# EnzoCording/FleetRL

Measured on AMD Instinct MI355X. Metric: env-steps/sec (num_envs x EVs batch, 1 launch per step), higher is better.
Workload: dtype f64

## Files before the change

### fleetrl_amd/_capi.py

```python
from __future__ import annotations

import ctypes as C
import os

import numpy as np

ABI_VERSION = 11

OK, ERR_INVALID, ERR_HIP, ERR_STATE, ERR_NODEVICE, ERR_UNSUPPORTED = 0, 1, 2, 3, 4, 5
DEG_NONE, DEG_LINEAR, DEG_RAINFLOW = 0, 1, 2
PICK_STATIC, PICK_RANDOM, PICK_EVAL = 0, 1, 2
ACT_F32, ACT_F64 = 0, 1
LAUNCH_EAGER, LAUNCH_GRAPH, LAUNCH_DIRECT, LAUNCH_DIRECT_ONE_QUEUE = 0, 1, 2, 3
POLICY_UNCONTROLLED, POLICY_DISTRIBUTED, POLICY_NIGHT = 2, 3, 4
LP_UNREACHABLE, LP_NEG_RETURN, LP_ABOVE_TARGET, LP_GRID_NEGATIVE = 1, 2, 4, 8

DEVERR_OBS_FORMAT, DEVERR_NEG_LIFE, DEVERR_SOH_MISMATCH, DEVERR_DOD_RANGE, DEVERR_TABLE_END, DEVERR_INTERNAL, DEVERR_PLACEMENT = 1, 2, 4, 8, 16, 32, 64

FIELDS = {
    "soc": (0, np.float64, True),
    "hours_left": (1, np.float32, True),
    "soh": (2, np.float64, True),
    "soc_deg": (3, np.float64, True),
    "target_soc": (4, np.float64, True),
# ... 516 lines not shown
    lib.fleet_rccl_comm_create.argtypes = [C.c_int, C.c_int, C.c_int, vp, C.POINTER(vp)]
    lib.fleet_rccl_comm_destroy.argtypes = [vp]
    lib.fleet_gather_episode_stats_rccl.argtypes = [vp, vp, C.c_int, vp]
    if hasattr(lib, "fleet_direct_queues"):
        lib.fleet_direct_queues.argtypes = [vp]
        lib.fleet_direct_queues.restype = C.c_int
    if hasattr(lib, "fleet_direct_placement"):
        lib.fleet_direct_placement.argtypes = [vp, C.POINTER(C.c_int32), C.POINTER(C.c_int32), C.POINTER(C.c_int32)]
        lib.fleet_direct_split_plan.argtypes = [C.c_uint32, C.c_int, C.POINTER(C.c_uint32)]
        lib.fleet_debug_direct_fault.argtypes = [vp, C.c_int, C.c_int]
        for name in ("fleet_direct_placement", "fleet_direct_split_plan", "fleet_debug_direct_fault"):
            getattr(lib, name).restype = C.c_int
    if hasattr(lib, "fleet_step_instance"):
        lib.fleet_step_instance.argtypes = [C.c_int] * 8 + [C.c_char_p, C.c_size_t, C.POINTER(C.c_uint32)]
        lib.fleet_step_instance.restype = C.c_int
        lib.fleet_max_evs_per_lane_group.argtypes = []
        lib.fleet_max_evs_per_lane_group.restype = C.c_int
    if hasattr(lib, "fleet_set_direct_state_only"):
        lib.fleet_set_direct_state_only.argtypes = [vp, C.c_int]
        lib.fleet_direct_packet_counts.argtypes = [vp, C.POINTER(C.c_uint64), C.POINTER(C.c_uint64)]
        lib.fleet_step_has_state_only.argtypes = [C.c_int] * 8 + [C.POINTER(C.c_int32)]
        for name in ("fleet_set_direct_state_only", "fleet_direct_packet_counts", "fleet_step_has_state_only"):
            getattr(lib, name).restype = C.c_int
    if hasattr(lib, "fleet_selftest_stress"):
        lib.fleet_selftest_stress.argtypes = [C.c_int, C.c_uint64, C.c_uint64, C.POINTER(C.c_double)]
        lib.fleet_selftest_stress.restype = C.c_int
    if hasattr(lib, "fleet_selftest_division"):
        lib.fleet_selftest_division.argtypes = [C.c_int, C.c_uint64, C.c_uint64, C.POINTER(C.c_uint64)]
        lib.fleet_selftest_division.restype = C.c_int
    lib.fleet_state_layout.argtypes = [C.POINTER(FleetParams), C.POINTER(FleetStateLayout)]
    lib.fleet_state_table_hash.argtypes = [C.POINTER(FleetParams), C.POINTER(FleetTablesC), C.POINTER(C.c_uint64)]
    lib.fleet_state_check.argtypes = [C.POINTER(FleetParams), C.c_uint64, vp, C.c_uint64]
    lib.fleet_state_bytes.argtypes = [vp, C.POINTER(C.c_uint64)]
    for name in ("fleet_state_save_dev", "fleet_state_load_dev", "fleet_state_save_host", "fleet_state_load_host"):
        getattr(lib, name).argtypes = [vp, vp, C.c_uint64]
    lib.fleet_fork_envs.argtypes = [vp, vp, vp, vp, C.c_int]
    for name in STATE_SYMBOLS:
        getattr(lib, name).restype = C.c_int
    dp = C.POINTER(C.c_double)
    lib.fleet_norm_create.argtypes = [C.c_int, C.POINTER(FleetNormParams), C.POINTER(vp)]
    lib.fleet_norm_destroy.argtypes = [vp]
    lib.fleet_norm_last_error.argtypes = [vp]
    lib.fleet_norm_set_stream.argtypes = [vp, vp]
    lib.fleet_norm_configure.argtypes = [vp, C.POINTER(FleetNormParams)]
    lib.fleet_norm_reset_dev.argtypes = [vp, f32p, f32p]
    lib.fleet_norm_step_dev.argtypes = [vp, f32p, f64p, u8p, f32p, f32p, f64p, f32p]
# ... 227 lines not shown
SACTRAIN_SYMBOLS = ("fleet_sactrain_create", "fleet_sactrain_destroy", "fleet_sactrain_last_error", "fleet_sactrain_describe",
                    "fleet_sactrain_alpha_dev", "fleet_sactrain_scale_dev", "fleet_sactrain_polyak_dev", "fleet_sactrain_sac_dev")

COLLECT_SYMBOLS = ("fleet_collect_create", "fleet_collect_destroy", "fleet_collect_last_error", "fleet_collect_describe",
                   "fleet_collect_reset_dev", "fleet_collect_ppo_dev", "fleet_collect_offpolicy_dev", "fleet_collect_episodes_dev",
                   "fleet_collect_finish_dev", "fleet_collect_episodes_read")

EVAL_SYMBOLS = ("fleet_eval_create", "fleet_eval_destroy", "fleet_eval_last_error", "fleet_eval_describe", "fleet_eval_sync_norm_dev",
                "fleet_eval_run_dev", "fleet_eval_episodes_dev", "fleet_eval_clear_dev", "fleet_eval_best_load_dev", "fleet_eval_best_export_dev",
                "fleet_eval_episodes_read")

EXPORTED_SYMBOLS = (
    "fleet_obs_dim", "fleet_create", "fleet_destroy", "fleet_last_error", "fleet_set_stream", "fleet_get_stream", "fleet_use_own_stream",
    "fleet_synchronize", "fleet_stream_query", "fleet_log_capacity", "fleet_log_dropped", "fleet_log_read", "fleet_log_clear",
    "fleet_log_summary_dev", "fleet_set_start_schedule", "fleet_reset_dev", "fleet_step_dev", "fleet_step_many_dev", "fleet_rollout_policy_dev",
    "fleet_set_night_policy", "fleet_reset_host",
    "fleet_step_host", "fleet_get", "fleet_get_dev", "fleet_get_dist_factor", "fleet_check_errors", "fleet_timer_start",
    "fleet_timer_stop", "fleet_timer_mark", "fleet_timer_read", "fleet_run_tape_dev", "fleet_time_steps_dev",
    "fleet_host_alloc", "fleet_host_free", "fleet_last_step_episodes", "fleet_last_step_error_bits",
    "fleet_time_regions_begin", "fleet_time_regions_read", "fleet_rccl_unique_id", "fleet_rccl_comm_create",
    "fleet_rccl_comm_destroy", "fleet_gather_episode_stats_rccl", "fleet_selftest_division", "fleet_direct_queues", "fleet_selftest_stress",
    "fleet_direct_placement", "fleet_direct_split_plan", "fleet_debug_direct_fault", "fleet_set_rainflow_count_all",
    "fleet_lp_plan_dev", "fleet_step_instance", "fleet_max_evs_per_lane_group",
    "fleet_set_direct_state_only", "fleet_direct_packet_counts", "fleet_step_has_state_only",
) + NORM_SYMBOLS + STATE_SYMBOLS + ROLLOUT_SYMBOLS + REPLAY_SYMBOLS + POLICY_SYMBOLS + EXPLORE_SYMBOLS + NOISE_SYMBOLS + QTARGET_SYMBOLS + PPO_SYMBOLS + TD3_SYMBOLS + ADAM_SYMBOLS + TRAIN_SYMBOLS + OFFPOLICY_SYMBOLS + SAC_SYMBOLS + COLLECT_SYMBOLS + EVAL_SYMBOLS


def step_instance(num_envs: int, num_cars: int, deg_mode: int, real_time: bool, log_data: bool, act_mode: int = ACT_F32, K: int = 1,
                  has_done_count: bool = False) -> tuple[str, int]:
    name = C.create_string_buffer(64)
    grid = C.c_uint32()
    rc = load_library().fleet_step_instance(int(num_envs), int(num_cars), int(deg_mode), int(bool(real_time)), int(bool(log_data)),
                                            int(act_mode), int(K), int(bool(has_done_count)), name, len(name), C.byref(grid))
    if rc != OK:
        raise FleetHipError(rc, "fleet_step_instance: argument out of range")
    return name.value.decode(), int(grid.value)


def step_has_state_only(num_envs: int, num_cars: int, deg_mode: int, real_time: bool, log_data: bool, act_mode: int = ACT_F32, K: int = 1,
                        has_done_count: bool = False) -> bool:
    out = C.c_int32()
    rc = load_library().fleet_step_has_state_only(int(num_envs), int(num_cars), int(deg_mode), int(bool(real_time)), int(bool(log_data)),
                                                  int(act_mode), int(K), int(bool(has_done_count)), C.byref(out))
    if rc != OK:
        raise FleetHipError(rc, "fleet_step_has_state_only: argument out of range")
    return bool(out.value)

# ... 116 lines not shown
```

### fleetrl_amd/batch.py

```python
from __future__ import annotations

import ctypes as C

import numpy as np

from . import _capi
from ._capi import FleetHipError

__all__ = ["FleetBatch", "FleetHipError"]


class _PinnedBuffer:

    _dead: list = []

    def __init__(self, lib, nbytes: int):
        out = C.c_void_p()
        rc = lib.fleet_host_alloc(int(nbytes), C.byref(out))
        if rc != _capi.OK or not out.value:
            raise FleetHipError(rc, "fleet_host_alloc failed")
        self._lib, self.address, self.nbytes = lib, int(out.value), int(nbytes)

    def array(self, shape, dtype) -> np.ndarray:
        raw = (C.c_char * self.nbytes).from_address(self.address)
# ... 244 lines not shown
    def set_rainflow_count_all(self, on: bool = True):
        self._check(self.lib.fleet_set_rainflow_count_all(self.h, 1 if on else 0))

    def run_tape_dev(self, steps: int, tape_ptr: int, tape_len: int, obs_ptr: int, reward_ptr: int, done_ptr: int,
                     use_graph: bool = True, act_dtype: int = _capi.ACT_F32):
        self._check(self.lib.fleet_run_tape_dev(self.h, int(steps), tape_ptr, int(tape_len), act_dtype, obs_ptr,
                                                 reward_ptr, done_ptr, int(use_graph)))

    def direct_placement(self):
        m = (C.c_int32 * 8)()
        nx, ag = C.c_int32(), C.c_int32()
        self._check(self.lib.fleet_direct_placement(self.h, m, C.byref(nx), C.byref(ag)))
        return [int(x) for x in m], int(nx.value), bool(ag.value)

    def debug_direct_fault(self, kind: int, tape_row: int):
        self._check(self.lib.fleet_debug_direct_fault(self.h, int(kind), int(tape_row)))

    def direct_queues(self) -> int:
        return int(self.lib.fleet_direct_queues(self.h)) if hasattr(self.lib, "fleet_direct_queues") else 0

    def set_direct_state_only(self, on: bool = True):
        self._check(self.lib.fleet_set_direct_state_only(self.h, 1 if on else 0))

    def direct_packet_counts(self) -> tuple[int, int]:
        live, dead = C.c_uint64(), C.c_uint64()
        self._check(self.lib.fleet_direct_packet_counts(self.h, C.byref(live), C.byref(dead)))
        return int(live.value), int(dead.value)

    def time_steps_dev(self, steps: int, tape_ptr: int, tape_len: int, obs_ptr: int, reward_ptr: int, done_ptr: int,
                       act_dtype: int = _capi.ACT_F32) -> np.ndarray:
        ms = np.zeros(int(steps), dtype=np.float32)
        self._check(self.lib.fleet_time_steps_dev(self.h, int(steps), tape_ptr, int(tape_len), act_dtype, obs_ptr,
                                                   reward_ptr, done_ptr, ms.ctypes.data))
        return ms

    def time_regions_begin(self, regions: int, steps: int, tape_ptr: int, tape_len: int, obs_ptr: int, reward_ptr: int, done_ptr: int,
                           use_graph: bool = True, act_dtype: int = _capi.ACT_F32):
        self._n_regions = int(regions)
        self._check(self.lib.fleet_time_regions_begin(self.h, int(regions), int(steps), tape_ptr, int(tape_len), act_dtype, obs_ptr,
                                                       reward_ptr, done_ptr, int(use_graph)))

    def time_regions_read(self) -> np.ndarray:
        ms = np.zeros(self._n_regions, dtype=np.float32)
        self._check(self.lib.fleet_time_regions_read(self.h, ms.ctypes.data))
        return ms

# ... 89 lines not shown
```

### fleetrl_amd/csrc/fleet_batch.h

```cpp
#pragma once
#include <hip/hip_runtime.h>
#include <stdint.h>

#include <string>
#include <tuple>
#include <vector>

#include "fleet_device.h"
#include "fleet_direct.h"
#include "fleet_state.h"

struct TapeKey {
  const void* tape = nullptr;
  int len = 0, dtype = 0;
  float* obs = nullptr;
  float* term = nullptr;
  double* reward = nullptr;
  uint8_t* done = nullptr;
  int mode = 0;
  uint64_t gen = 0;
  bool operator==(const TapeKey& o) const {
    return std::tie(tape, len, dtype, obs, term, reward, done, mode, gen) ==
           std::tie(o.tape, o.len, o.dtype, o.obs, o.term, o.reward, o.done, o.mode, o.gen);
  }
// ... 31 lines not shown
  char* pin_small = nullptr;
  void* pin_actions = nullptr;
  float* pin_term = nullptr;
  char* pin_obs = nullptr;
  static constexpr int kObsPieces = 3;
  hipEvent_t obs_piece_ev[kObsPieces] = {};
  bool host_step_has_episodes = false;
  uint32_t last_step_err = 0;
  double* st_dist = nullptr;
  int32_t* dev_sched = nullptr;
  FleetCold cold_host{};
  FleetCold* cold_dev = nullptr;
  FleetDev* self_dev = nullptr;
  void* st_field = nullptr;
  hipEvent_t ev_start = nullptr, ev_stop = nullptr;
  std::vector<hipEvent_t> region_events;
  hipGraphExec_t graph_exec = nullptr;
  TapeKey graph_key;
  FleetDirect* direct = nullptr;
  TapeKey dq_key;
  bool dq_timed = false;
  std::vector<double> dq_spans_us;
  bool direct_state_only = true;
  uint64_t gen = 1;
  void* lp_scratch = nullptr;
  size_t lp_scratch_bytes = 0;
  void* logsum_scratch = nullptr;
  uint64_t table_hash = 0;
  FleetStateHeader* pin_state_hdr = nullptr;
  FleetForkScratch fork;
};

inline int direct_drain(FleetEnvBatch* h) {
  if (!h || !h->direct) return FLEET_OK;
  return fleet_direct_wait(h->direct, &h->dq_spans_us, &h->error);
}
#define FLEET_ENTER(h)                          \
  do {                                          \
    const int _rc = direct_drain(h);            \
    if (_rc != FLEET_OK) return _rc;            \
  } while (0)

#define HIP_TRY(b, expr)                                                                         \
  do {                                                                                           \
    hipError_t _e = (expr);                                                                      \
    if (_e != hipSuccess) {                                                                      \
// ... 40 lines not shown
```

### fleetrl_amd/csrc/fleet_capi.hip

```cpp
#include <algorithm>
#include <cstdio>
#include <cstring>

#include "fleet_batch.h"
#include "fleet_logsum.h"
#include "fleet_lp.h"

static thread_local std::string g_create_error;

static const char* deverr_names(uint32_t bits, char* buf, size_t n) {
  snprintf(buf, n, "%s%s%s%s%s%s%s",
           (bits & FLEET_DEVERR_PLACEMENT) ? " placement: a workgroup of a run on the library's own queue ran on another die than probed, the run's results are void;" : "",
           (bits & FLEET_DEVERR_INTERNAL) ? " internal: inconsistent launch arguments;" : "",
           (bits & FLEET_DEVERR_OBS_FORMAT) ? " observation format not recognized;" : "",
           (bits & FLEET_DEVERR_NEG_LIFE) ? " life degradation is negative;" : "",
           (bits & FLEET_DEVERR_SOH_MISMATCH) ? " degradation calculation is not correct;" : "",
           (bits & FLEET_DEVERR_DOD_RANGE) ? " DoD too large;" : "",
           (bits & FLEET_DEVERR_TABLE_END) ? " the episode runs past the last table row;" : "");
  return buf;
}

void fleet_set_create_error(const std::string& why) { g_create_error = why; }

template <typename Edit>
static int push_cold(fleet_handle h, Edit edit) {
  h->gen += 1;
  HIP_TRY(h, hipSetDevice(h->device));
  HIP_TRY(h, hipStreamSynchronize(h->stream));
  const int rc = edit();
  if (rc != FLEET_OK) return rc;
  HIP_TRY(h, hipMemcpy(h->cold_dev, &h->cold_host, sizeof(FleetCold), hipMemcpyHostToDevice));
  return FLEET_OK;
}

extern "C" {

int fleet_obs_dim(const FleetParams* p) {
  if (!p || p->num_cars < 1) return -1;
  return fleet_obs_dim_of(p);
}

int fleet_create(const FleetParams* p, const FleetTables* t, int device, fleet_handle* out) {
  if (out) *out = nullptr;
  if (const char* why = fleet_validate(p, t)) {
    g_create_error = why;
    return FLEET_ERR_INVALID;
  }
  if (!out) {
    g_create_error = "null output handle";
    return FLEET_ERR_INVALID;
  }
  FleetEnvBatch* b = new FleetEnvBatch();
  int rc = fleet_create_impl(p, t, device, b);
// ... 82 lines not shown
  return push_cold(h, [&]() -> int {
    if (h->dev_sched) {
      (void)hipFree(h->dev_sched);
      h->dev_sched = nullptr;
    }
    h->cold_host.sched = nullptr;
    h->cold_host.sched_n = 0;
    if (n_episodes > 0) {
      const size_t n = (size_t)n_episodes * h->d.E;
      for (size_t i = 0; i < n; ++i)
        if (starts[i] < 0 || starts[i] > h->d.T - 1) {
          h->error = "start row outside the table";
          return FLEET_ERR_INVALID;
        }
      HIP_TRY(h, hipMalloc((void**)&h->dev_sched, n * sizeof(int32_t)));
      HIP_TRY(h, hipMemcpy(h->dev_sched, starts, n * sizeof(int32_t), hipMemcpyHostToDevice));
      h->cold_host.sched = h->dev_sched;
      h->cold_host.sched_n = n_episodes;
    }
    return FLEET_OK;
  });
}

int fleet_reset_dev(fleet_handle h, const uint8_t* mask, float* obs) {
  FLEET_ENTER(h);
  if (!h || !obs) return FLEET_ERR_INVALID;
  HIP_TRY(h, hipSetDevice(h->device));
  HIP_TRY(h, fleet_launch_reset(h->d, mask, obs, h->stream));
  return FLEET_OK;
}

int fleet_step_dev(fleet_handle h, const void* actions, int act_dtype, float* obs, double* reward, uint8_t* done,
                   float* terminal_obs) {
  FLEET_ENTER(h);
  if (!h || !actions || !obs || !reward || !done || !act_dtype_ok(act_dtype)) {
    if (h) h->error = "fleet_step_dev: null buffer or bad action dtype";
    return FLEET_ERR_INVALID;
  }
  HIP_TRY(h, hipSetDevice(h->device));
  HIP_TRY(h, fleet_launch_step(h->d, actions, act_dtype, 1, obs, reward, done, terminal_obs, nullptr, h->stream));
  return FLEET_OK;
}

int fleet_step_many_dev(fleet_handle h, int K, const void* actions, int act_dtype, float* obs, double* reward_sum,
                        int32_t* done_count) {
  FLEET_ENTER(h);
// ... 298 lines not shown
    char names[400], buf[640];
    snprintf(buf, sizeof buf, "%s: the handle has device error bits raised (0x%x:%s) and its state is not saved or forked", who, any,
             deverr_names(any, names, sizeof names));
    h->error = buf;
    return FLEET_ERR_STATE;
  }
  return FLEET_OK;
}

static int state_save(fleet_handle h, void* blob, uint64_t bytes, bool host) {
  FLEET_ENTER(h);
  if (!h) return FLEET_ERR_INVALID;
  HIP_TRY(h, hipSetDevice(h->device));
  if (!h->pin_state_hdr) HIP_TRY(h, hipHostMalloc((void**)&h->pin_state_hdr, sizeof(FleetStateHeader), hipHostMallocDefault));
  const int rc = state_clean(h, host ? "fleet_state_save_host" : "fleet_state_save_dev");
  if (rc != FLEET_OK) return rc;
  return fleet_state_save(state_refs(h), blob, bytes, host);
}

static int state_load(fleet_handle h, const void* blob, uint64_t bytes, bool host) {
  FLEET_ENTER(h);
  if (!h) return FLEET_ERR_INVALID;
  HIP_TRY(h, hipSetDevice(h->device));
  const int rc = fleet_state_load(state_refs(h), blob, bytes, host);
  if (rc != FLEET_OK) return rc;
  h->gen += 1;
  h->host_step_has_episodes = false;
  h->last_step_err = 0;
  return FLEET_OK;
}

int fleet_state_bytes(fleet_handle h, uint64_t* bytes) {
  if (!h || !bytes) return FLEET_ERR_INVALID;
  *bytes = fleet_state_blob_bytes(state_refs(h));
  return FLEET_OK;
}
int fleet_state_save_dev(fleet_handle h, void* blob_dev, uint64_t bytes) { return state_save(h, blob_dev, bytes, false); }
int fleet_state_save_host(fleet_handle h, void* blob_host, uint64_t bytes) { return state_save(h, blob_host, bytes, true); }
int fleet_state_load_dev(fleet_handle h, const void* blob_dev, uint64_t bytes) { return state_load(h, blob_dev, bytes, false); }
int fleet_state_load_host(fleet_handle h, const void* blob_host, uint64_t bytes) { return state_load(h, blob_host, bytes, true); }

int fleet_fork_envs(fleet_handle dst, fleet_handle src, const int32_t* dst_idx_host, const int32_t* src_idx_host, int n) {
  FLEET_ENTER(dst);
  if (!dst || !src) return FLEET_ERR_INVALID;
  if (src != dst) {
    const int rc = direct_drain(src);
    if (rc != FLEET_OK) {
      dst->error = "fleet_fork_envs: the source handle: " + src->error;
      return rc;
    }
  }
  if (dst->device != src->device) {
    dst->error = "fleet_fork_envs: the two handles are on different devices";
    return FLEET_ERR_INVALID;
  }
  if (dst->d.log_pos || src->d.log_pos) {
    dst->error = "fleet_fork_envs: a handle with the data log on is not forked (log_data = 1)";
    return FLEET_ERR_UNSUPPORTED;
  }
  HIP_TRY(dst, hipSetDevice(dst->device));
  int rc = state_clean(dst, "fleet_fork_envs");
  if (rc != FLEET_OK) return rc;
  if (src != dst && (rc = state_clean(src, "fleet_fork_envs")) != FLEET_OK) {
    dst->error = src->error;
    return rc;
  }
  return fleet_state_fork(state_refs(dst), state_refs(src), src == dst, dst_idx_host, src_idx_host, n, &dst->fork);
}

}

static int selftest_run(int device, uint64_t n, uint64_t seed, void* out, size_t words,
                        hipError_t (*launch)(unsigned long long, unsigned long long, unsigned long long*, hipStream_t)) {
  if (!out || n == 0) return FLEET_ERR_INVALID;
  int ndev = 0;
  if (hipGetDeviceCount(&ndev) != hipSuccess || ndev <= 0) return FLEET_ERR_NODEVICE;
  if (device < 0 || device >= ndev) return FLEET_ERR_INVALID;
  if (hipSetDevice(device) != hipSuccess) return FLEET_ERR_HIP;
  unsigned long long* dev = nullptr;
  unsigned long long host[2] = {0, 0};
  const size_t bytes = words * sizeof host[0];
  if (hipMalloc(&dev, bytes) != hipSuccess) return FLEET_ERR_HIP;
  int rc = FLEET_OK;
  if (hipMemset(dev, 0, bytes) != hipSuccess || launch(n, seed, dev, nullptr) != hipSuccess ||
      hipMemcpy(host, dev, bytes, hipMemcpyDeviceToHost) != hipSuccess)
    rc = FLEET_ERR_HIP;
  (void)hipFree(dev);
  memcpy(out, host, bytes);
  return rc;
}
// ... 9 lines not shown
```

### fleetrl_amd/csrc/fleet_device.h

```cpp
#pragma once
#include <hip/hip_runtime.h>
#include <stdint.h>

#include "../../include/fleet_hip.h"

struct PhysRow {
  double k_cost;
  double k_rev;
  double k_charge;
  double k_discharge;
  double load;
  double pv;
  double pv_share;
  uint32_t flags_next;
  uint32_t pad;
  double dt;
};

struct SegRec {
  double sor;
  uint32_t tlx;
  uint32_t se;
};
#define SEG_RAW 0x40000000u
// ... 82 lines not shown
  double fd_cyc;
  double fd_cal;
  double sei_l;
  double sei_soh;
};
struct FleetCold {
  double min_laxity, def_soc, init_soh, temperature, dt;
  double batt_cap_nominal, hn_denominator, max_soc, max_hours_needed, max_laxity;
  double inv_max_soc, inv_max_hours_needed, inv_max_laxity;
  unsigned long long seed;
  int picker_mode, start_lo, start_hi, env_id_offset;
  int sched_n;
  int normalize;
  const int32_t* sched;
  const int32_t* pick_rows;
  const uint16_t* tab_hm;
  int32_t* night_start;
  int night_hour, night_minute;
  int night_limit_s;
  int step_s;
  const int32_t* tab_last_deg;
  int32_t* last_len;
  int rf_count_all;
};
#define FLEET_NIGHT_IDLE INT32_MIN

struct FleetDev {
  int E, N, T;
  int obs_dim;
  int episode_steps;
  int stack_cap;
  int tail_a_len;
  int tail_b_len;
  int tail_stride;
  int aux, normalize, is_caretaker, deg_mode, auto_reset;
  int real_time;
  int carry_run;
  double dt, p_avail, init_cap, eta_c, eta_d, penalty_invalid, penalty_oc, clip_oc, target_soc, target_soc_lunch, eps,
      fully_charged_reward, evse_power, grid_connection, penalty_overload, max_time_left, stress_temp;
  double hn_scale;
  double inv_eta_c;
  const SegRec* seg;
  const PhysRow* tab_phys;
  const uint8_t* tab_flags;
  const float* tab_tail;
  const int32_t* tab_finish;
  const FleetCold* cold;
  const struct FleetDev* self;
  Hot* hot;
  SegRec* run;
  double* soh;
  double* soc_deg;
  SeiRec* sei;
  EnvRec* env;
  uint32_t* err_any;
  int log_cap;
  int32_t* log_pos;
  int32_t* log_row;
  double* log_env;
  double* log_ev;
  float* log_obs;
  double* rf_rows;
  int rf_row_stride;
};

hipError_t fleet_launch_reset(const FleetDev& d, const uint8_t* mask, float* obs, hipStream_t s);
hipError_t fleet_launch_step(const FleetDev& d, const void* actions, int act_dtype, int K, float* obs, double* reward,
                             uint8_t* done, float* terminal_obs, int32_t* done_count, hipStream_t s);
struct FleetStepLaunch {
  const void* host_fn;
  const void* host_fn_dead;
  unsigned grid, block, args_bytes;
  unsigned actions_offset[2];
  unsigned packed_n_offset;
  unsigned guard_offset;
  unsigned rec_offset;
  unsigned dead_offset;
  alignas(8) unsigned char args[640];
};
struct FleetStepInstance {
  int G, deg;
  bool multi, wide, log, a64;
  int mode;
};
int fleet_describe_step_instance(const FleetDev& d, int act_mode, int K, bool has_done_count, char* name, size_t name_bytes,
                                 unsigned* grid);
// ... 11 lines not shown
```

### fleetrl_amd/csrc/fleet_kernels.hip

```cpp
#include "fleet_device.h"
#include <cstddef>

#include "fleet_stamps.h"

namespace {

constexpr int kSingleWaves = 4, kMultiWaves = 4, kMultiWideWaves = 2;
#ifndef FLEET_KBLOCK
#define FLEET_KBLOCK 256
#endif
constexpr int kBlock = FLEET_KBLOCK;
constexpr int kMaxGroup = 256;
static_assert(kMaxGroup <= kBlock && kBlock % 64 == 0, "a lane group is a whole number of a workgroup's wavefronts");

}

#include "fleet_wave.h"
#include "fleet_obs.h"
#include "fleet_rainflow.h"
#include "fleet_reset.h"

namespace {

template <int DEG, bool WIDE>
// ... 267 lines not shown
    night_st = d.cold->night_start[e];
    if (G >= 64) night_st = __builtin_amdgcn_readfirstlane(night_st);
  }

  static_assert(!LOG || MULTI, "the data log is compiled into the multi-step kernel only");
  constexpr bool log_on = LOG;
  int lp = log_on ? d.log_pos[e] : 0;
  if (G >= 64) lp = __builtin_amdgcn_readfirstlane(lp);

  const bool rt = kRt && (d.real_time != 0);
  constexpr bool kRfCarry = MULTI && !WIDE && DEG == FLEET_DEG_RAINFLOW;
  RfAccHead acc_c = {0.0, 0, 0};
  RfTop top_c = {0.0, 0.0};
  auto carry_load = [&]() {
    const EvIx i0 = {(size_t)e * N, (unsigned)(g < N ? g : N - 1)};
    const double* row = rf_row_of(d, i0);
    acc_c = *reinterpret_cast<const RfAccHead*>(row);
    top_c = *reinterpret_cast<const RfTop*>(row + 2);
  };
  if (kRfCarry) carry_load();
  double last_rew = 0.0;
  bool last_done = false;
  uint32_t head_after = 0;
  bool head_reset = false;
  for (int k = 0; rt || k < steps; ++k) {
    const int t = r.t;
    int t1 = t + 1;
    if (t1 > d.T - 1) { t1 = d.T - 1; err |= FLEET_DEVERR_TABLE_END; }
    const int t2 = t1 + 1 > d.T - 1 ? d.T - 1 : t1 + 1;
    const bool is_done = (t + 1 == r.t_end);
    const bool done_now = is_done || (!d.auto_reset && (uint32_t)(t + 1) > (uint32_t)r.t_end);
    const bool resets = is_done && d.auto_reset;
    const bool rf_live = MULTI ? (t < rf_until) : head_live;
    float* const step_row = resets ? term_row : obs_row;
    const bool write_step_obs = obs_live && env_ok && (step_row != nullptr) && (!MULTI || rt || resets || k == steps - 1);

    FLEET_STAMP(1);
    const PhysHot ph = *reinterpret_cast<const PhysHot*>(d.tab_phys + (t + ((kEarly || DEG != FLEET_DEG_RAINFLOW) ? vzero : 0)));
    uint32_t flags_after = 0;
    if (kEarly) flags_after = reinterpret_cast<const PhysHot*>(d.tab_phys + (t1 + vzero))->flags_next;
    const double dt_step = rt ? d.tab_phys[t].dt : d.dt;
    const uint32_t flags1 = kEarly ? head_flags : ph.flags_next;
    const bool lunch = d.is_caretaker && (flags1 & FLEET_TFLAG_LUNCH);
    const bool deg_row = (DEG != FLEET_DEG_NONE) && (flags1 & FLEET_TFLAG_DEG);
    if (!MULTI && G >= 64 && ((DEG == FLEET_DEG_RAINFLOW && deg_row) || is_done)) __builtin_amdgcn_s_setprio(3);
    const size_t abase = ((size_t)(rt ? 0 : k) * d.E + e) * N;

// ... 257 lines not shown
          soh_new = d.soh[i] - deg;
        }
        d.soh[i] = soh_new;
        if (logs) {
          double* lev = d.log_ev + lrow * 4 * N + c;
          lev[2 * N] = deg;
          lev[3 * N] = soh_new;
        }
        if (!WIDE) break;
      }
    }
    if (logs) lp += 1;
    head_after = flags_after;
    if (is_done) {
      n_done += 1;
      if (leader && env_ok) {
        EnvRec* er = d.env + e;
        er->last_ep_return = ep_return;
        d.cold->last_len[e] = ep_len;
        er->start_done |= (int32_t)0x80000000u;
      }
      r.episodes += 1;
      if (kTailB ? (lt.auto_reset != 0) : resets) {
        head_reset = true;
        if (env_ok) {
          if constexpr (kStateOnly) reset_env<G, LOG>(*d.self, e, g, leader, r, obs_live ? obs_row : nullptr, lp, rf_until);
          else reset_env<G, LOG>(*d.self, e, g, leader, r, obs_row, lp, rf_until);
          if (kRfCarry) carry_load();
        } else {
          r.t = choose_start(d.cold, d.E, e, r.episodes);
          r.t_end = d.tab_finish ? d.tab_finish[r.t] : r.t + d.episode_steps;
          r.nsamp = (DEG != FLEET_DEG_NONE) ? 1 : 0;
        }
        ep_return = 0.0;
        ep_len = 0;
        penalty_record = 0.0;
        if constexpr (kTailC) {
          head_after = d.tab_phys[r.t].flags_next;
          asm volatile("" : "+v"(head_after));
        }
      }
    }
    last_done = done_now;
    if (rt) {
      const int hm1 = d.cold->tab_hm[t1];
      const bool minute15 = ((hm1 & 255) == 15) && !(hm1 & 0x8000);
      if (group_any<G>(ev_lane) || is_done || minute15 || (t + 1 > d.T - 1)) break;
    }
    }
  }

  {
  const FleetDev& d = kTailB ? late_args_same() : late_args();
  if (!kEarly && (!WIDE || d.carry_run) && env_ok) {
    const int rn = r.t + 1 > d.T - 1 ? d.T - 1 : r.t + 1;
    for (int c = g; c < N; c += G) d.run[(size_t)e * N + c] = d.seg[(size_t)rn * N + c];
  }
  if (leader && env_ok) {
    EnvRec* er = kTailC ? p_env + e : d.env + e;
    uint32_t nflags = head_after;
    if (!kEarly || (head_reset && !kTailC)) nflags = d.tab_phys[r.t].flags_next;
    r.nsamp = HEAD_PACK(r.nsamp, nflags, r.t < rf_until);
    er->h = r;
    er->ep_return = ep_return;
    er->ep_len = ep_len;
    er->penalty_record = penalty_record;
    if (log_on) d.log_pos[e] = lp;
    if (MULTI) {
      reward[e] = rt ? last_rew : reward_sum;
      if (done && (rt || steps == 1)) done[e] = last_done ? 1 : 0;
      if (done_count) done_count[e] = n_done;
      if (kPol && act_mode == FLEET_ACT_POLICY_NIGHT) d.cold->night_start[e] = night_st;
    }
  }
  if constexpr (!MULTI) {
    typedef TwinLateTail Tail;
    static_assert(offsetof(StepKernargs, rec_blocks) == offsetof(StepKernargs, guard_bytes) + 8, "one 24-byte piece of the argument block");
    Tail tl_b = {lt.rec, lt.blocks, lt.rows, lt.rotate};
    karg_ptr kp = nullptr;
    if constexpr (!kTailB) {
      kp = (karg_ptr)__builtin_amdgcn_kernarg_segment_ptr() + offsetof(StepKernargs, guard_bytes);
      asm volatile("" : "+s"(kp));
    }
    const Tail& tl = kTailB ? tl_b : *(const Tail*)(const __attribute__((address_space(4))) Tail*)kp;
// ... 38 lines not shown
```

### fleetrl_amd/csrc/fleet_reset.h

```cpp
#pragma once
#include "fleet_device.h"
#include "fleet_obs.h"
#include "fleet_rainflow.h"
#include "fleet_wave.h"

namespace {

__device__ __forceinline__ void reset_ev(const FleetDev& d, int e, int c, int start, float* __restrict__ obs_row,
                                         float* __restrict__ log_obs_row, double* __restrict__ log_ev) {
  const int N = d.N;
  const FleetCold* cd = d.cold;
  const int next = start + 1 > d.T - 1 ? d.T - 1 : start + 1;
  const EvIx ix = {(size_t)e * N, (unsigned)c};
  const size_t i = ix.flat();
  const SegRec s0 = d.seg[(size_t)start * N + c];
  d.run[i] = d.seg[(size_t)next * N + c];
  const RowRec tb = seg_row(s0, start, d.dt);
  const bool t090 = HOT_T090(d.hot[i].bits);
  const double soh = 1.0 * cd->init_soh;
  const double cap = soh * d.init_cap;
  double soc = tb.sor;
  const float hl = tb.tl;
  const double tgt = t090 ? 0.9 : d.target_soc;
  const double time_needed = (tgt - soc) * cap / d.p_avail;
// ... 2 lines not shown
  const double soc_deg = (soc == 0.0) ? cd->def_soc : soc;
  d.hot[i] = hot_encode(d, ix, soc, soc_deg, hl, 1, 0, tb.there, t090, false);
  d.soh[i] = soh;
  if (d.deg_mode == FLEET_DEG_RAINFLOW) {
    RfHdr* hp = reinterpret_cast<RfHdr*>(d.rf_rows + i * (size_t)d.rf_row_stride);
    RfHdr hd = *hp;
    hd.mean_sum = 0.0;
    hd.csum = 0.0;
    hd.nc = 0;
    hd.s1 = 0.0;
    hd.s2 = soc_deg;
    *hp = hd;
  }
  if (obs_row) write_obs_ev(d, obs_row, c, soc, hl, tgt, tb);
  if (log_obs_row) {
    write_obs_ev(d, log_obs_row, c, soc, hl, tgt, tb);
    double* lev = log_ev + c;
    lev[0] = 0.0;
    lev[N] = 0.0;
    lev[2 * N] = 0.0;
    lev[3 * N] = soh;
  }
}
__device__ __forceinline__ int reset_times(const FleetDev& d, int e, EnvHead& r, int& rf_until) {
  const FleetCold* cd = d.cold;
  const int start = choose_start(cd, d.E, e, r.episodes);
  r.t = start;
  r.t_end = d.tab_finish ? d.tab_finish[start] : start + d.episode_steps;
  r.nsamp = (d.deg_mode != FLEET_DEG_NONE) ? 1 : 0;
  const int last = cd->tab_last_deg[r.t_end > d.T - 1 ? d.T - 1 : r.t_end];
  rf_until = (cd->rf_count_all || !d.auto_reset) ? INT32_MAX : (last > start ? last : -1);
  return start;
}
__device__ __forceinline__ void reset_head(const FleetDev& d, int e, const EnvHead& r, int start, int rf_until) {
  EnvRec* er = d.env + e;
  EnvHead hd = r;
  hd.nsamp = HEAD_PACK(r.nsamp, d.tab_phys[start].flags_next, start < rf_until);
  er->h = hd;
  er->rf_until = rf_until;
  er->ep_return = 0.0;
  er->ep_len = 0;
  er->penalty_record = 0.0;
  er->start_done = start;
}

template <int G, bool LOG>
__device__ __forceinline__ void reset_env(const FleetDev& d, int e, int g, bool leader, EnvHead& r, float* __restrict__ obs_row, int& lp,
                                          int& rf_until) {
  const bool log_on = LOG && (d.log_pos != nullptr);
  const int N = d.N;
  const int start = reset_times(d, e, r, rf_until);
  const size_t lrow = log_on ? (size_t)(lp % d.log_cap) * d.E + e : 0;
  float* const log_obs_row = log_on ? d.log_obs + lrow * d.obs_dim : nullptr;
  double* const log_ev = log_on ? d.log_ev + lrow * 4 * N : nullptr;
  for (int c = g; c < N; c += G) reset_ev(d, e, c, start, obs_row, log_obs_row, log_ev);
  if (obs_row) write_obs_tail<G>(d, obs_row, start, g);
  if (log_on) {
    write_obs_tail<G>(d, log_obs_row, start, g);
    if (leader) {
      d.log_row[lrow] = (int32_t)((uint32_t)start | 0x80000000u);
      double* le = d.log_env + lrow * 4;
      le[0] = le[1] = le[2] = le[3] = 0.0;
    }
    lp += 1;
  }
  if (leader) reset_head(d, e, r, start, rf_until);
}

template <int G>
__global__ __launch_bounds__(kBlock) void fleet_reset_kernel(FleetDev d, const uint8_t* __restrict__ mask, float* __restrict__ obs) {
  const int g = threadIdx.x % G;
  const int e = blockIdx.x * (kBlock / G) + threadIdx.x / G;
  if (e >= d.E) return;
  if (mask && !mask[e]) return;
  EnvHead r = d.env[e].h;
  r.nsamp = HEAD_NSAMP(r.nsamp);
  if (d.env[e].ep_len > 0 && d.env[e].start_done >= 0) r.episodes += 1;
  int lp = d.log_pos ? d.log_pos[e] : 0;
  int rf_until;
  reset_env<G, true>(d, e, g, g == G - 1, r, obs ? obs + (size_t)e * d.obs_dim : nullptr, lp, rf_until);
  if (d.log_pos && g == G - 1) d.log_pos[e] = lp;
}

}
```

### fleetrl_amd/csrc/fleet_tables.hip

```cpp
#include <cmath>
#include <cstring>

#include "fleet_batch.h"

int fleet_obs_dim_of(const FleetParams* p) {
  const int N = p->num_cars, L = p->price_lookahead, B = p->bl_pv_lookahead;
  int dim = 2 * N + (L + 1) * 2;
  if (p->include_building && p->include_pv)
    dim += 2 * (B + 1);
  else if (p->include_building || p->include_pv)
    dim += B + 1;
  if (p->aux) {
    dim += 5 * N + 1 + 6;
    if (p->include_building) dim += 3;
  }
  return dim;
}

const char* fleet_validate(const FleetParams* p, const FleetTables* t) {
  if (!p || !t) return "null params/tables";
  if (p->abi_version != FLEET_ABI_VERSION) return "abi_version mismatch";
  if (p->struct_bytes != (int)sizeof(FleetParams)) return "FleetParams size mismatch";
  if (p->num_envs < 1 || p->num_cars < 1 || p->table_rows < 2) return "num_envs/num_cars/table_rows out of range";
  if (p->num_cars > 65535) return "num_cars: at most 65535 EVs per env";
// ... 218 lines not shown
  d.real_time = p->real_time ? 1 : 0;
  d.carry_run = (N <= fleet_max_evs_per_lane_group()) ? 1 : 0;
  d.dt = p->dt; d.evse_power = p->evse_power;
  d.p_avail = p->obc_max_power < p->evse_power ? p->obc_max_power : p->evse_power;
  d.init_cap = p->init_battery_cap; d.grid_connection = p->grid_connection;
  d.eta_c = p->charging_eff; d.eta_d = p->discharging_eff;
  d.stress_temp = std::exp(6.93E-2 * (p->temperature - 25.0) * ((25.0 + 273.15) / (p->temperature + 273.15)));
  d.penalty_invalid = p->penalty_invalid_action; d.penalty_oc = p->penalty_overcharging; d.clip_oc = p->clip_overcharging;
  d.penalty_overload = p->penalty_overloading; d.fully_charged_reward = p->fully_charged_reward;
  d.target_soc = p->target_soc; d.target_soc_lunch = p->target_soc_lunch; d.eps = p->eps;
  d.max_time_left = p->max_time_left;
  d.hn_scale = p->batt_cap_nominal / (p->evse_power * p->charging_eff);
  d.inv_eta_c = 1.0 / p->charging_eff;

  FleetCold& cd = b->cold_host;
  cd.min_laxity = p->min_laxity; cd.def_soc = p->def_soc; cd.init_soh = p->init_soh; cd.temperature = p->temperature;
  cd.dt = p->dt; cd.batt_cap_nominal = p->batt_cap_nominal; cd.hn_denominator = p->evse_power * p->charging_eff;
  cd.max_soc = p->max_soc; cd.max_hours_needed = p->max_hours_needed; cd.max_laxity = p->max_laxity;
  cd.inv_max_soc = p->normalize ? 1.0 / p->max_soc : 1.0;
  cd.inv_max_hours_needed = p->normalize ? 1.0 / p->max_hours_needed : 1.0;
  cd.inv_max_laxity = p->normalize ? 1.0 / p->max_laxity : 1.0;
  cd.seed = p->seed; cd.picker_mode = p->picker_mode; cd.start_lo = p->start_lo; cd.start_hi = p->start_hi;
  cd.env_id_offset = p->env_id_offset; cd.sched_n = 0; cd.normalize = p->normalize; cd.sched = nullptr;

  int rc;
  {
    std::vector<PhysRow> phys;
    std::vector<uint8_t> flags;
    build_phys_rows(*p, *t, phys, flags);
    std::vector<float> tail;
    build_tail_rows(*p, *t, d.tail_a_len, d.tail_b_len, d.tail_stride, tail);
    std::vector<SegRec> seg;
    build_seg_rows(*p, *t, seg);
    if ((rc = dev_upload(b, &d.seg, seg.data(), seg.size()))) return rc;
    if ((rc = dev_upload(b, &d.tab_phys, phys.data(), phys.size()))) return rc;
    if ((rc = dev_upload(b, &d.tab_flags, flags.data(), flags.size()))) return rc;
    std::vector<int32_t> last_deg((size_t)T);
    int32_t last = -1;
    for (int r = 0; r < T; ++r) {
      if (flags[r] & FLEET_TFLAG_DEG) last = r;
      last_deg[r] = last;
    }
    if ((rc = dev_upload(b, &cd.tab_last_deg, last_deg.data(), last_deg.size()))) return rc;
    if ((rc = dev_upload(b, &d.tab_tail, tail.data(), tail.size()))) return rc;
    HIP_TRY(b, hipStreamSynchronize(b->stream));
  }
// ... 17 lines not shown
    if ((rc = dev_upload(b, &d.tab_finish, t->finish_row, (size_t)T))) return rc;
    HIP_TRY(b, hipStreamSynchronize(b->stream));
  }
  if ((rc = dev_alloc(b, &b->cold_dev, 1))) return rc;
  HIP_TRY(b, hipMemcpyAsync(b->cold_dev, &cd, sizeof(FleetCold), hipMemcpyHostToDevice, b->stream));
  d.cold = b->cold_dev;

  const size_t EN = (size_t)E * N;
  if ((rc = dev_alloc(b, &d.hot, EN))) return rc;
  if ((rc = dev_alloc(b, &d.run, EN))) return rc;
  if ((rc = dev_alloc(b, &d.soh, EN))) return rc;
  if ((rc = dev_alloc(b, &d.soc_deg, EN))) return rc;
  if ((rc = dev_alloc(b, &d.sei, EN))) return rc;
  if (p->log_data) {
    d.log_cap = p->log_capacity > 0 ? p->log_capacity : 2 * (p->episode_steps + 1);
    const size_t rows = (size_t)d.log_cap * E;
    if ((rc = dev_alloc(b, &d.log_pos, (size_t)E))) return rc;
    if ((rc = dev_alloc(b, &d.log_row, rows))) return rc;
    if ((rc = dev_alloc(b, &d.log_env, rows * 4))) return rc;
    if ((rc = dev_alloc(b, &d.log_ev, rows * 4 * N))) return rc;
    if ((rc = dev_alloc(b, &d.log_obs, rows * (size_t)d.obs_dim))) return rc;
  }
  if ((rc = dev_alloc(b, &d.env, E))) return rc;
  if (p->deg_mode == FLEET_DEG_RAINFLOW) {
    d.rf_row_stride = ((RF_HDR_WORDS + d.stack_cap + 15) / 16) * 16;
    if ((uint64_t)N * (uint64_t)d.rf_row_stride * 8ull >= (1ull << 32)) {
      b->error = "num_cars x episode length: the rainflow rows of one env exceed 4 GiB";
      return FLEET_ERR_INVALID;
    }
    if ((rc = dev_alloc(b, &d.rf_rows, EN * (size_t)d.rf_row_stride, false))) return rc;
    RfHdr h0;
    memset(&h0, 0, sizeof h0);
    h0.rf_len = 1;
    std::vector<RfHdr> hdrs(EN, h0);
    HIP_TRY(b, hipMemcpy2DAsync(d.rf_rows, (size_t)d.rf_row_stride * 8, hdrs.data(), sizeof(RfHdr), sizeof(RfHdr), EN,
                                hipMemcpyHostToDevice, b->stream));
    HIP_TRY(b, hipStreamSynchronize(b->stream));
  }
  {
    std::vector<double> soh(EN, p->init_soh);
    std::vector<SeiRec> sei(EN);
    for (auto& q : sei) { q.fd_cyc = 0; q.fd_cal = 0; q.sei_soh = p->init_soh; q.sei_l = 1.0 - p->init_soh; }
    HIP_TRY(b, hipMemcpyAsync(d.soh, soh.data(), EN * sizeof(double), hipMemcpyHostToDevice, b->stream));
    HIP_TRY(b, hipMemcpyAsync(d.sei, sei.data(), EN * sizeof(SeiRec), hipMemcpyHostToDevice, b->stream));
    HIP_TRY(b, hipStreamSynchronize(b->stream));
  }
// ... 23 lines not shown
```

### include/fleet_hip.h

```cpp
#ifndef FLEET_HIP_H
#define FLEET_HIP_H

#include <stddef.h>
#include <stdint.h>

#ifdef __cplusplus
extern "C" {
#endif

#define FLEET_ABI_VERSION 11
#define FLEET_API __attribute__((visibility("default")))

#define FLEET_OK 0
#define FLEET_ERR_INVALID 1
#define FLEET_ERR_HIP 2
#define FLEET_ERR_STATE 3
#define FLEET_ERR_NODEVICE 4
#define FLEET_ERR_UNSUPPORTED 5

#define FLEET_DEG_NONE 0
#define FLEET_DEG_LINEAR 1
#define FLEET_DEG_RAINFLOW 2

#define FLEET_PICK_STATIC 0
// ... 269 lines not shown

int fleet_timer_start(fleet_handle h);
int fleet_timer_stop(fleet_handle h, float* elapsed_ms);
int fleet_timer_mark(fleet_handle h);
int fleet_timer_read(fleet_handle h, float* elapsed_ms);
#define FLEET_LAUNCH_EAGER 0
#define FLEET_LAUNCH_GRAPH 1
#define FLEET_LAUNCH_DIRECT 2
#define FLEET_LAUNCH_DIRECT_ONE_QUEUE 3
int fleet_run_tape_dev(fleet_handle h, int steps, const void* tape, int tape_len, int act_dtype,
                       float* obs, double* reward, uint8_t* done, int use_graph);

int fleet_direct_queues(fleet_handle h);

int fleet_direct_placement(fleet_handle h, int32_t map8[8], int32_t* num_xcc, int32_t* any_grid);
int fleet_direct_split_plan(uint32_t grid_workgroups, int split, uint32_t part_grid[2]);
int fleet_step_instance(int num_envs, int num_cars, int deg_mode, int real_time, int log_data, int act_mode, int K,
                        int has_done_count, char* name, size_t name_bytes, uint32_t* grid);
int fleet_max_evs_per_lane_group(void);
int fleet_set_direct_state_only(fleet_handle h, int on);
int fleet_direct_packet_counts(fleet_handle h, uint64_t* live, uint64_t* state_only);
int fleet_step_has_state_only(int num_envs, int num_cars, int deg_mode, int real_time, int log_data, int act_mode, int K,
                              int has_done_count, int32_t* has_twin);
int fleet_debug_direct_fault(fleet_handle h, int kind, int tape_row);

int fleet_time_regions_begin(fleet_handle h, int regions, int steps, const void* tape, int tape_len, int act_dtype,
                             float* obs, double* reward, uint8_t* done, int use_graph);
int fleet_time_regions_read(fleet_handle h, float* region_ms);

int fleet_time_steps_dev(fleet_handle h, int steps, const void* tape, int tape_len, int act_dtype, float* obs,
                         double* reward, uint8_t* done, float* per_launch_ms);

int fleet_selftest_division(int device, uint64_t n_pairs, uint64_t seed, uint64_t* mismatches);
int fleet_selftest_stress(int device, uint64_t n_samples, uint64_t seed, double* max_rel_err);

typedef struct FleetNormParams {
  int32_t struct_bytes;
  int32_t num_envs;
  int32_t obs_dim;
  int32_t training, norm_obs, norm_reward;
  double clip_obs, clip_reward;
  double gamma;
  double epsilon;
} FleetNormParams;
typedef struct FleetNorm* fleet_norm_handle;

// ... 743 lines not shown
```

Before: 813.4 million.

## Precompute next-episode reset times per env to shorten auto-reset path

Adds a per-env 32-byte EnvNext record holding the next episode's start, end, rainflow cutoff and head flags. It is written at each reset and read at the next auto-reset, guarded by a generation counter that is bumped on cold edits, state loads and forks. This removes the dependent choose_start, table and last-degradation lookups from the critical path of a reset inside the step kernel. In exchange each reset does an extra record read, computes the following episode's times, and adds new invalidation logic that must stay consistent.

```diff
diff --git a/fleetrl_amd/_capi.py b/fleetrl_amd/_capi.py
--- a/fleetrl_amd/_capi.py
+++ b/fleetrl_amd/_capi.py
@@ -562,6 +562,9 @@
         lib.fleet_step_has_state_only.argtypes = [C.c_int] * 8 + [C.POINTER(C.c_int32)]
         for name in ("fleet_set_direct_state_only", "fleet_direct_packet_counts", "fleet_step_has_state_only"):
             getattr(lib, name).restype = C.c_int
+    if hasattr(lib, "fleet_set_reset_precompute"):
+        lib.fleet_set_reset_precompute.argtypes = [vp, C.c_int]
+        lib.fleet_set_reset_precompute.restype = C.c_int
     if hasattr(lib, "fleet_selftest_stress"):
         lib.fleet_selftest_stress.argtypes = [C.c_int, C.c_uint64, C.c_uint64, C.POINTER(C.c_double)]
         lib.fleet_selftest_stress.restype = C.c_int
@@ -835,7 +838,7 @@
     "fleet_rccl_comm_destroy", "fleet_gather_episode_stats_rccl", "fleet_selftest_division", "fleet_direct_queues", "fleet_selftest_stress",
     "fleet_direct_placement", "fleet_direct_split_plan", "fleet_debug_direct_fault", "fleet_set_rainflow_count_all",
     "fleet_lp_plan_dev", "fleet_step_instance", "fleet_max_evs_per_lane_group",
-    "fleet_set_direct_state_only", "fleet_direct_packet_counts", "fleet_step_has_state_only",
+    "fleet_set_direct_state_only", "fleet_direct_packet_counts", "fleet_step_has_state_only", "fleet_set_reset_precompute",
 ) + NORM_SYMBOLS + STATE_SYMBOLS + ROLLOUT_SYMBOLS + REPLAY_SYMBOLS + POLICY_SYMBOLS + EXPLORE_SYMBOLS + NOISE_SYMBOLS + QTARGET_SYMBOLS + PPO_SYMBOLS + TD3_SYMBOLS + ADAM_SYMBOLS + TRAIN_SYMBOLS + OFFPOLICY_SYMBOLS + SAC_SYMBOLS + COLLECT_SYMBOLS + EVAL_SYMBOLS
 
 
diff --git a/fleetrl_amd/batch.py b/fleetrl_amd/batch.py
--- a/fleetrl_amd/batch.py
+++ b/fleetrl_amd/batch.py
@@ -290,6 +290,9 @@
     def set_direct_state_only(self, on: bool = True):
         self._check(self.lib.fleet_set_direct_state_only(self.h, 1 if on else 0))
 
+    def set_reset_precompute(self, on: bool = True):
+        self._check(self.lib.fleet_set_reset_precompute(self.h, 1 if on else 0))
+
     def direct_packet_counts(self) -> tuple[int, int]:
         live, dead = C.c_uint64(), C.c_uint64()
         self._check(self.lib.fleet_direct_packet_counts(self.h, C.byref(live), C.byref(dead)))
diff --git a/fleetrl_amd/csrc/fleet_batch.h b/fleetrl_amd/csrc/fleet_batch.h
--- a/fleetrl_amd/csrc/fleet_batch.h
+++ b/fleetrl_amd/csrc/fleet_batch.h
@@ -77,6 +77,7 @@
   bool dq_timed = false;
   std::vector<double> dq_spans_us;
   bool direct_state_only = true;
+  bool reset_precompute = true;
   uint64_t gen = 1;
   void* lp_scratch = nullptr;
   size_t lp_scratch_bytes = 0;
diff --git a/fleetrl_amd/csrc/fleet_capi.hip b/fleetrl_amd/csrc/fleet_capi.hip
--- a/fleetrl_amd/csrc/fleet_capi.hip
+++ b/fleetrl_amd/csrc/fleet_capi.hip
@@ -29,6 +29,7 @@
   HIP_TRY(h, hipStreamSynchronize(h->stream));
   const int rc = edit();
   if (rc != FLEET_OK) return rc;
+  fleet_cold_next_gen(h->cold_host, h->reset_precompute);
   HIP_TRY(h, hipMemcpy(h->cold_dev, &h->cold_host, sizeof(FleetCold), hipMemcpyHostToDevice));
   return FLEET_OK;
 }
@@ -157,6 +158,16 @@
   });
 }
 
+int fleet_set_reset_precompute(fleet_handle h, int on) {
+  FLEET_ENTER(h);
+  if (!h) return FLEET_ERR_INVALID;
+  if (h->reset_precompute == (on != 0)) return FLEET_OK;
+  return push_cold(h, [&]() -> int {
+    h->reset_precompute = (on != 0);
+    return FLEET_OK;
+  });
+}
+
 int fleet_reset_dev(fleet_handle h, const uint8_t* mask, float* obs) {
   FLEET_ENTER(h);
   if (!h || !obs) return FLEET_ERR_INVALID;
@@ -501,8 +512,12 @@
   FLEET_ENTER(h);
   if (!h) return FLEET_ERR_INVALID;
   HIP_TRY(h, hipSetDevice(h->device));
+  fleet_cold_next_gen(h->cold_host, h->reset_precompute);
   const int rc = fleet_state_load(state_refs(h), blob, bytes, host);
-  if (rc != FLEET_OK) return rc;
+  if (rc != FLEET_OK) {
+    (void)hipMemcpy(h->cold_dev, &h->cold_host, sizeof(FleetCold), hipMemcpyHostToDevice);
+    return rc;
+  }
   h->gen += 1;
   h->host_step_has_episodes = false;
   h->last_step_err = 0;
@@ -544,7 +559,11 @@
     dst->error = src->error;
     return rc;
   }
-  return fleet_state_fork(state_refs(dst), state_refs(src), src == dst, dst_idx_host, src_idx_host, n, &dst->fork);
+  rc = fleet_state_fork(state_refs(dst), state_refs(src), src == dst, dst_idx_host, src_idx_host, n, &dst->fork);
+  if (rc != FLEET_OK || n == 0) return rc;
+  fleet_cold_next_gen(dst->cold_host, dst->reset_precompute);
+  HIP_TRY(dst, hipMemcpyAsync(dst->cold_dev, &dst->cold_host, sizeof(FleetCold), hipMemcpyHostToDevice, dst->stream));
+  return FLEET_OK;
 }
 
 }
diff --git a/fleetrl_amd/csrc/fleet_device.h b/fleetrl_amd/csrc/fleet_device.h
--- a/fleetrl_amd/csrc/fleet_device.h
+++ b/fleetrl_amd/csrc/fleet_device.h
@@ -128,8 +128,25 @@
   const int32_t* tab_last_deg;
   int32_t* last_len;
   int rf_count_all;
+  uint32_t next_gen;
+  uint32_t next_gen_last;
 };
 #define FLEET_NIGHT_IDLE INT32_MIN
+inline void fleet_cold_next_gen(FleetCold& c, bool on) {
+  c.next_gen_last = c.next_gen_last + 1u ? c.next_gen_last + 1u : 1u;
+  c.next_gen = on ? c.next_gen_last : 0u;
+}
+
+struct EnvNext {
+  int32_t start;
+  int32_t t_end;
+  int32_t rf_until;
+  uint32_t flags;
+  int32_t episode;
+  uint32_t gen;
+  uint32_t pad[2];
+};
+static_assert(sizeof(EnvNext) == 32, "one 32-byte record per env");
 
 struct FleetDev {
   int E, N, T;
@@ -168,6 +185,7 @@
   float* log_obs;
   double* rf_rows;
   int rf_row_stride;
+  EnvNext* env_next;
 };
 
 hipError_t fleet_launch_reset(const FleetDev& d, const uint8_t* mask, float* obs, hipStream_t s);
diff --git a/fleetrl_amd/csrc/fleet_kernels.hip b/fleetrl_amd/csrc/fleet_kernels.hip
--- a/fleetrl_amd/csrc/fleet_kernels.hip
+++ b/fleetrl_amd/csrc/fleet_kernels.hip
@@ -313,7 +313,6 @@
   double last_rew = 0.0;
   bool last_done = false;
   uint32_t head_after = 0;
-  bool head_reset = false;
   for (int k = 0; rt || k < steps; ++k) {
     const int t = r.t;
     int t1 = t + 1;
@@ -617,10 +616,14 @@
       }
       r.episodes += 1;
       if (kTailB ? (lt.auto_reset != 0) : resets) {
-        head_reset = true;
         if (env_ok) {
-          if constexpr (kStateOnly) reset_env<G, LOG>(*d.self, e, g, leader, r, obs_live ? obs_row : nullptr, lp, rf_until);
-          else reset_env<G, LOG>(*d.self, e, g, leader, r, obs_row, lp, rf_until);
+          karg_ptr rkp = (karg_ptr)__builtin_amdgcn_kernarg_segment_ptr() + offsetof(StepKernargPrefix, d_arg);
+          if constexpr (kEarly) asm volatile("" : "+s"(rkp));
+          const FleetDev& dr = kEarly ? *(const FleetDev*)(const __attribute__((address_space(4))) FleetDev*)rkp : *d.self;
+          uint32_t rflags = 0;
+          if constexpr (kStateOnly) reset_env<G, LOG, true>(dr, e, g, leader, r, obs_live ? obs_row : nullptr, lp, rf_until, rflags);
+          else reset_env<G, LOG, true>(dr, e, g, leader, r, obs_row, lp, rf_until, rflags);
+          if (kEarly) head_after = rflags;
           if (kRfCarry) carry_load();
         } else {
           r.t = choose_start(d.cold, d.E, e, r.episodes);
@@ -630,10 +633,6 @@
         ep_return = 0.0;
         ep_len = 0;
         penalty_record = 0.0;
-        if constexpr (kTailC) {
-          head_after = d.tab_phys[r.t].flags_next;
-          asm volatile("" : "+v"(head_after));
-        }
       }
     }
     last_done = done_now;
@@ -654,7 +653,7 @@
   if (leader && env_ok) {
     EnvRec* er = kTailC ? p_env + e : d.env + e;
     uint32_t nflags = head_after;
-    if (!kEarly || (head_reset && !kTailC)) nflags = d.tab_phys[r.t].flags_next;
+    if (!kEarly) nflags = d.tab_phys[r.t].flags_next;
     r.nsamp = HEAD_PACK(r.nsamp, nflags, r.t < rf_until);
     er->h = r;
     er->ep_return = ep_return;
diff --git a/fleetrl_amd/csrc/fleet_reset.h b/fleetrl_amd/csrc/fleet_reset.h
--- a/fleetrl_amd/csrc/fleet_reset.h
+++ b/fleetrl_amd/csrc/fleet_reset.h
@@ -48,20 +48,22 @@
     lev[3 * N] = soh;
   }
 }
-__device__ __forceinline__ int reset_times(const FleetDev& d, int e, EnvHead& r, int& rf_until) {
-  const FleetCold* cd = d.cold;
-  const int start = choose_start(cd, d.E, e, r.episodes);
-  r.t = start;
-  r.t_end = d.tab_finish ? d.tab_finish[start] : start + d.episode_steps;
-  r.nsamp = (d.deg_mode != FLEET_DEG_NONE) ? 1 : 0;
-  const int last = cd->tab_last_deg[r.t_end > d.T - 1 ? d.T - 1 : r.t_end];
-  rf_until = (cd->rf_count_all || !d.auto_reset) ? INT32_MAX : (last > start ? last : -1);
-  return start;
+__device__ __forceinline__ EnvNext episode_times(const FleetDev& d, const FleetCold* cd, int e, int episode, uint32_t gen) {
+  EnvNext n;
+  const int start = choose_start(cd, d.E, e, episode);
+  n.start = start;
+  n.t_end = d.tab_finish ? d.tab_finish[start] : start + d.episode_steps;
+  const int last = cd->tab_last_deg[n.t_end > d.T - 1 ? d.T - 1 : n.t_end];
+  n.rf_until = (cd->rf_count_all || !d.auto_reset) ? INT32_MAX : (last > start ? last : -1);
+  n.flags = d.tab_phys[start].flags_next;
+  n.episode = episode;
+  n.gen = gen;
+  return n;
 }
-__device__ __forceinline__ void reset_head(const FleetDev& d, int e, const EnvHead& r, int start, int rf_until) {
+__device__ __forceinline__ void reset_head(const FleetDev& d, int e, const EnvHead& r, int start, int rf_until, uint32_t flags) {
   EnvRec* er = d.env + e;
   EnvHead hd = r;
-  hd.nsamp = HEAD_PACK(r.nsamp, d.tab_phys[start].flags_next, start < rf_until);
+  hd.nsamp = HEAD_PACK(r.nsamp, flags, start < rf_until);
   er->h = hd;
   er->rf_until = rf_until;
   er->ep_return = 0.0;
@@ -70,12 +72,43 @@
   er->start_done = start;
 }
 
-template <int G, bool LOG>
+template <int G, bool LOG, bool USE_NEXT>
 __device__ __forceinline__ void reset_env(const FleetDev& d, int e, int g, bool leader, EnvHead& r, float* __restrict__ obs_row, int& lp,
-                                          int& rf_until) {
+                                          int& rf_until, uint32_t& flags) {
   const bool log_on = LOG && (d.log_pos != nullptr);
   const int N = d.N;
-  const int start = reset_times(d, e, r, rf_until);
+  const FleetCold* cd = d.cold;
+  const uint32_t gen = cd->next_gen;
+  EnvNext cur;
+  bool hit = false;
+  if (USE_NEXT) {
+    int vz = 0;
+    asm volatile("" : "+v"(vz));
+    const uint4* rec = reinterpret_cast<const uint4*>(d.env_next + (e + vz));
+    const uint4 w0 = rec[0];
+    const uint2 w1 = *reinterpret_cast<const uint2*>(rec + 1);
+    auto uni = [](uint32_t v) -> uint32_t { return G >= 64 ? (uint32_t)__builtin_amdgcn_readfirstlane((int)v) : v; };
+    cur.start = (int32_t)uni(w0.x);
+    cur.t_end = (int32_t)uni(w0.y);
+    cur.rf_until = (int32_t)uni(w0.z);
+    cur.flags = uni(w0.w);
+    cur.episode = (int32_t)uni(w1.x);
+    cur.gen = uni(w1.y);
+    hit = (gen != 0u) && (cur.gen == gen) && (cur.episode == r.episodes);
+  }
+  if (!hit) cur = episode_times(d, cd, e, r.episodes, gen);
+  int start = cur.start;
+  r.t_end = cur.t_end;
+  rf_until = cur.rf_until;
+  flags = cur.flags;
+  if (G >= 64) {
+    start = __builtin_amdgcn_readfirstlane(start);
+    r.t_end = __builtin_amdgcn_readfirstlane(r.t_end);
+    rf_until = __builtin_amdgcn_readfirstlane(rf_until);
+    flags = (uint32_t)__builtin_amdgcn_readfirstlane((int)flags);
+  }
+  r.t = start;
+  r.nsamp = (d.deg_mode != FLEET_DEG_NONE) ? 1 : 0;
   const size_t lrow = log_on ? (size_t)(lp % d.log_cap) * d.E + e : 0;
   float* const log_obs_row = log_on ? d.log_obs + lrow * d.obs_dim : nullptr;
   double* const log_ev = log_on ? d.log_ev + lrow * 4 * N : nullptr;
@@ -90,7 +123,15 @@
     }
     lp += 1;
   }
-  if (leader) reset_head(d, e, r, start, rf_until);
+  if (leader) reset_head(d, e, r, start, rf_until, flags);
+  if (gen != 0u) {
+    const EnvNext nxt = episode_times(d, cd, e, r.episodes + 1, gen);
+    if (leader) {
+      uint4* rec = reinterpret_cast<uint4*>(d.env_next + e);
+      rec[0] = make_uint4((uint32_t)nxt.start, (uint32_t)nxt.t_end, (uint32_t)nxt.rf_until, nxt.flags);
+      *reinterpret_cast<uint2*>(rec + 1) = make_uint2((uint32_t)nxt.episode, nxt.gen);
+    }
+  }
 }
 
 template <int G>
@@ -104,7 +145,8 @@
   if (d.env[e].ep_len > 0 && d.env[e].start_done >= 0) r.episodes += 1;
   int lp = d.log_pos ? d.log_pos[e] : 0;
   int rf_until;
-  reset_env<G, true>(d, e, g, g == G - 1, r, obs ? obs + (size_t)e * d.obs_dim : nullptr, lp, rf_until);
+  uint32_t flags;
+  reset_env<G, true, false>(d, e, g, g == G - 1, r, obs ? obs + (size_t)e * d.obs_dim : nullptr, lp, rf_until, flags);
   if (d.log_pos && g == G - 1) d.log_pos[e] = lp;
 }
 
diff --git a/fleetrl_amd/csrc/fleet_tables.hip b/fleetrl_amd/csrc/fleet_tables.hip
--- a/fleetrl_amd/csrc/fleet_tables.hip
+++ b/fleetrl_amd/csrc/fleet_tables.hip
@@ -264,6 +264,7 @@
   cd.inv_max_laxity = p->normalize ? 1.0 / p->max_laxity : 1.0;
   cd.seed = p->seed; cd.picker_mode = p->picker_mode; cd.start_lo = p->start_lo; cd.start_hi = p->start_hi;
   cd.env_id_offset = p->env_id_offset; cd.sched_n = 0; cd.normalize = p->normalize; cd.sched = nullptr;
+  cd.next_gen = cd.next_gen_last = 1u;
 
   int rc;
   {
@@ -327,6 +328,7 @@
     if ((rc = dev_alloc(b, &d.log_obs, rows * (size_t)d.obs_dim))) return rc;
   }
   if ((rc = dev_alloc(b, &d.env, E))) return rc;
+  if ((rc = dev_alloc(b, &d.env_next, E))) return rc;
   if (p->deg_mode == FLEET_DEG_RAINFLOW) {
     d.rf_row_stride = ((RF_HDR_WORDS + d.stack_cap + 15) / 16) * 16;
     if ((uint64_t)N * (uint64_t)d.rf_row_stride * 8ull >= (1ull << 32)) {
diff --git a/include/fleet_hip.h b/include/fleet_hip.h
--- a/include/fleet_hip.h
+++ b/include/fleet_hip.h
@@ -315,6 +315,7 @@
 int fleet_direct_packet_counts(fleet_handle h, uint64_t* live, uint64_t* state_only);
 int fleet_step_has_state_only(int num_envs, int num_cars, int deg_mode, int real_time, int log_data, int act_mode, int K,
                               int has_done_count, int32_t* has_twin);
+int fleet_set_reset_precompute(fleet_handle h, int on);
 int fleet_debug_direct_fault(fleet_handle h, int kind, int tape_row);
 
 int fleet_time_regions_begin(fleet_handle h, int regions, int steps, const void* tape, int tape_len, int act_dtype,
```

New measurement: 813.7 million, median of 2. Within noise of the previous version (+0.0%).
